# CodyRichter/MLMicroserviceTemplate

Hardware: AMD Instinct MI355X
Metric: requests/sec (whole node) + p50 latency, ResNet-50 bs=32 (higher is better)
Workload: dtype bf16; 1 GPU; model=resnet50-v1.5, global_batch=32, per_gpu_batch=32, image_size=224, parallelism=dp1, backend=fused, concurrent_slots=True, cu_partitions=2, hipgraph=True, inflight=4, numa_bound=True, partition_mode=intra, prestage=False, ranks_consistent=True, dist_backend=none, dist_world=1

## Files before the change

### mlmicroservicetemplate_amd/models/resnet.py

```python
from __future__ import annotations

import math
import os
from dataclasses import dataclass
from typing import Dict, List, Optional, Tuple

import torch
import torch.nn.functional as F

STAGES: Tuple[Tuple[int, int, int, int], ...] = (
    (3, 64, 256, 1),
    (4, 128, 512, 2),
    (6, 256, 1024, 2),
    (3, 512, 2048, 2),
)
IMAGENET_MEAN = (0.485 * 255, 0.456 * 255, 0.406 * 255)
IMAGENET_STD = (0.229 * 255, 0.224 * 255, 0.225 * 255)
NUM_CLASSES = 1000


@dataclass
class ConvSpec:
    name: str
    cin: int
    cout: int
    k: int
    stride: int
    pad: int


def conv_specs() -> List[ConvSpec]:
    specs = [ConvSpec("stem", 3, 64, 7, 2, 3)]
    cin = 64
    for si, (nblocks, mid, cout, stride) in enumerate(STAGES):
        for bi in range(nblocks):
            s = stride if bi == 0 else 1
            p = f"layer{si + 1}.{bi}"
            specs.append(ConvSpec(p + ".conv1", cin, mid, 1, 1, 0))
            specs.append(ConvSpec(p + ".conv2", mid, mid, 3, s, 1))
            specs.append(ConvSpec(p + ".conv3", mid, cout, 1, 1, 0))
            if bi == 0:
                specs.append(ConvSpec(p + ".down", cin, cout, 1, s, 0))
            cin = cout
    return specs


def init_resnet50(seed: int = 0, num_classes: int = NUM_CLASSES) -> Dict[str, torch.Tensor]:
    g = torch.Generator().manual_seed(seed)
    params: Dict[str, torch.Tensor] = {}
    for spec in conv_specs():
        fan_in = spec.cin * spec.k * spec.k
# ... 190 lines not shown
    for s, _hin, ho in conv_shapes(image_size):
        total += 2.0 * ho * ho * s.cout * s.cin * s.k * s.k
    return total + 2.0 * 2048 * NUM_CLASSES


class ResNet50Fused:

    def __init__(self, params: Dict[str, torch.Tensor], device, max_batch: int = 256,
                 tuning: Optional[Dict[str, Tuple[int, int]]] = None, image_size: int = 224):
        from .. import ops

        self.ops = ops
        self.device = torch.device(device)
        self.image_size = image_size
        self.tuning = dict(tuning or {})
        self.specs = {s.name: s for s in conv_specs()}
        self.w: Dict[str, torch.Tensor] = {}
        self.b: Dict[str, torch.Tensor] = {}
        for s in conv_specs():
            scale, bias = fold_bn(params, s.name)
            w = params[s.name + ".w"] * scale.view(-1, 1, 1, 1)
            self.w[s.name] = ops.pack_conv_weight(w).to(self.device)
            self.b[s.name] = bias.to(device=self.device, dtype=torch.float32).contiguous()
        self.dual_w: Dict[str, torch.Tensor] = {}
        self.dual_b: Dict[str, torch.Tensor] = {}
        for si, (_nb, _m, _c, _s) in enumerate(STAGES):
            p0 = f"layer{si + 1}.0"
            w3, wd = self.w[p0 + ".conv3"], self.w[p0 + ".down"]
            self.dual_w[p0] = torch.cat([w3.reshape(w3.shape[0], -1), wd.reshape(wd.shape[0], -1)], 1).contiguous()
            self.dual_b[p0] = (self.b[p0 + ".conv3"] + self.b[p0 + ".down"]).contiguous()
        self.fuse_down = True
        self.chain = os.environ.get("MLS_CHAIN", "1") != "0"
        self.chain_skip: set = {b for b in os.environ.get("MLS_CHAIN_SKIP", "").split(",") if b}
        self.chain_l3 = os.environ.get("MLS_CHAIN_L3", "0") == "1"
        if os.environ.get("MLS_CHAIN_L2_CW"):
            ops.set_chain_l2_cw(int(os.environ["MLS_CHAIN_L2_CW"]))
        if os.environ.get("MLS_CHAIN_L2_BM"):
            ops.lib().mls_chain_set_l2_bm(int(os.environ["MLS_CHAIN_L2_BM"]))
        if os.environ.get("MLS_CHAIN_VARIANT"):
            ops.lib().mls_chain_set_variant(int(os.environ["MLS_CHAIN_VARIANT"]))
        self.fuse_stem = image_size == 224 and os.environ.get("MLS_FUSED_STEM", "1") != "0"
        self.fuse_stem_conv1 = os.environ.get("MLS_STEM_CONV1", "0") == "1"
        self.fc_w = params["fc.w"].to(device=self.device, dtype=torch.bfloat16).contiguous()
        self.fc_b = params["fc.b"].to(device=self.device, dtype=torch.float32).contiguous()
        self.num_classes = self.fc_w.shape[0]
        self.mean = IMAGENET_MEAN
        self.std = IMAGENET_STD
        self.max_batch = max_batch
        self._ws = ops.StreamWorkspace(self._workspace_bytes(max_batch) // 4 + 1, self.device)
        self.fuse_head = os.environ.get("MLS_FUSED_HEAD", "1") != "0"
        self._pool = ops.StreamWorkspace(max_batch * self.fc_w.shape[1], self.device, zero=True)

    @property
    def workspace(self) -> torch.Tensor:
        return self._ws.get()

    @torch.no_grad()
    def update_params(self, params: Dict[str, torch.Tensor]) -> None:
        from .. import ops

        for s in conv_specs():
            scale, bias = fold_bn(params, s.name)
            w = ops.pack_conv_weight(params[s.name + ".w"] * scale.view(-1, 1, 1, 1))
            self.w[s.name].copy_(w)
            self.b[s.name].copy_(bias)
        for si in range(len(STAGES)):
# ... 21 lines not shown
        return self.ops.gemm_heuristic(M, N, K)

    def _workspace_bytes(self, batch: int) -> int:
        need = 0
        for b in sorted({1, 2, 4, 8, 16, 32, 64, 128, 256, batch}):
            if b > batch:
                continue
            for name, M, N, K in self.layer_gemm_shapes(b):
                cfg, sk = self._plan(name, M, N, K)
                if cfg in self.ops.PIPE_CFGS:
                    sk = sk % 16 or 1
                if sk > 1:
                    need = max(need, sk * M * N * 4)
        return max(need, batch * NUM_CLASSES * 4, 1 << 20)

    def _conv(self, x, name, act, residual=None, pad=None):
        s = self.specs[name]
        cfg, sk = self.tuning.get(name, (0, 0))
        return self.ops.conv2d_nhwc(x, self.w[name], self.b[name], kernel=s.k, stride=s.stride,
                                    pad=s.pad if pad is None else pad,
                                    residual=residual, act=act, workspace=self.workspace, cfg=cfg, splitk=sk)


    def _chained(self, p: str, nxt: str, dual: bool) -> bool:
        if not self.chain or p in self.chain_skip:
            return False
        c3 = self.specs[p + ".conv3"]
        k = c3.cin + (self.specs[p + ".down"].cin if dual else 0)
        c1 = self.specs[nxt + ".conv1"]
        shape = (k, c3.cout, c1.cout)
        if shape == (256, 1024, 256) and not self.chain_l3:
            return False
        return c1.k == 1 and c1.stride == 1 and shape in self.ops.CHAIN_SHAPES

    def forward(self, images_u8_nhwc: torch.Tensor) -> torch.Tensor:
        ops = self.ops
        B = images_u8_nhwc.shape[0]
        if self.fuse_head:
            pooled = self._trunk(images_u8_nhwc, pool=True)
            _v, _i, logits = ops.fc_head(pooled, self.fc_w, self.fc_b, 0, logits=self._logits_buf(B))
            return logits.to(torch.bfloat16)
        x = self._trunk(images_u8_nhwc, pool=False)
        pooled = ops.avgpool_global_nhwc(x)
        cfg, sk = self.tuning.get("fc", (0, 0))
        return ops.gemm(pooled, self.fc_w, self.fc_b, workspace=self.workspace, cfg=cfg, splitk=sk)

    __call__ = forward

    def _logits_buf(self, B: int) -> torch.Tensor:
        return self.workspace[: B * self.num_classes].view(B, self.num_classes)

    def classify(self, images_u8_nhwc: torch.Tensor, k: int = 5, err: Optional[torch.Tensor] = None):
        if self.fuse_head:
            pooled = self._trunk(images_u8_nhwc, pool=True)
            B = images_u8_nhwc.shape[0]
            vals, idx, _ = self.ops.fc_head(pooled, self.fc_w, self.fc_b, k, logits=self._logits_buf(B), err=err)
            return vals, idx
        vals, idx = self.ops.softmax_topk(self.forward(images_u8_nhwc), k)
        if err is not None:
            bad = (err[: idx.shape[0]] != 0).view(-1, 1)
            idx = torch.where(bad, torch.full_like(idx, -1), idx)
            vals = torch.where(bad, torch.full_like(vals, float("nan")), vals)
        return vals, idx

    def _trunk(self, images_u8_nhwc: torch.Tensor, pool: bool) -> torch.Tensor:
        ops = self.ops
        B = images_u8_nhwc.shape[0]
        if B > self.max_batch:
            raise ValueError(f"batch {B} > max_batch {self.max_batch}")
        if self.fuse_stem and self.fuse_stem_conv1:
            x, t1 = ops.stem_pool_u8(images_u8_nhwc, self.w["stem"], self.b["stem"], self.mean, self.std,
                                     conv1_w=self.w["layer1.0.conv1"], conv1_b=self.b["layer1.0.conv1"])
        else:
            if self.fuse_stem:
                x = ops.stem_pool_u8(images_u8_nhwc, self.w["stem"], self.b["stem"], self.mean, self.std)
            else:
                x = ops.normalize_u8(images_u8_nhwc, self.mean, self.std, pad=3)
                x = self._conv(x, "stem", ops.ACT_RELU, pad=0)
                x = ops.maxpool2d_nhwc(x, 3, 2, 1)
            t1 = self._conv(x, "layer1.0.conv1", ops.ACT_RELU)
        blocks = [(si, bi) for si, (nblocks, _m, _c, _s) in enumerate(STAGES) for bi in range(nblocks)]
        for idx, (si, bi) in enumerate(blocks):
            p = f"layer{si + 1}.{bi}"
            nxt = f"layer{blocks[idx + 1][0] + 1}.{blocks[idx + 1][1]}" if idx + 1 < len(blocks) else None
            t2 = self._conv(t1, p + ".conv2", ops.ACT_RELU)
            dual = bi == 0 and self.fuse_down
            if nxt is not None and self._chained(p, nxt, dual):
                w1n, b1n = self.w[nxt + ".conv1"], self.b[nxt + ".conv1"]
                w1n = w1n.reshape(w1n.shape[0], -1)
                if dual:
                    x, t1 = ops.conv1x1_chain(t2, self.dual_w[p], self.dual_b[p], w1n, b1n, a2=x,
                                              stride2=self.specs[p + ".down"].stride)
                else:
                    w3 = self.w[p + ".conv3"]
                    x, t1 = ops.conv1x1_chain(t2, w3.reshape(w3.shape[0], -1), self.b[p + ".conv3"], w1n, b1n,
                                              residual=x)
                continue
            if dual:
                cfg, sk = self.tuning.get(p + ".dual", (0, 0))
                x = ops.conv1x1_dual(t2, x, self.dual_w[p], self.dual_b[p], stride2=self.specs[p + ".down"].stride,
                                     act=ops.ACT_RELU, workspace=self.workspace, cfg=cfg, splitk=sk)
            else:
                identity = self._conv(x, p + ".down", ops.ACT_NONE) if bi == 0 else x
                if nxt is None and pool:
                    pooled = self._pool.get()[: B * self.fc_w.shape[1]].view(B, -1)
                    cfg, _sk = self.tuning.get(p + ".conv3", (0, 0))
                    s3 = self.specs[p + ".conv3"]
                    ops.conv2d_pool(t2, self.w[p + ".conv3"], self.b[p + ".conv3"], pooled, kernel=s3.k,
                                    stride=s3.stride, pad=s3.pad, residual=identity, act=ops.ACT_RELU, cfg=cfg)
                    return pooled
                x = self._conv(t2, p + ".conv3", ops.ACT_RELU, residual=identity)
            if nxt is not None:
                t1 = self._conv(x, nxt + ".conv1", ops.ACT_RELU)
        if pool:
            pooled = self._pool.get()[: B * self.fc_w.shape[1]].view(B, -1)
            pooled.copy_(ops.avgpool_global_nhwc(x).float())
            return pooled
        return x
```

### mlmicroservicetemplate_amd/ops/__init__.py

```python
from __future__ import annotations

from . import _lib
from ._lib import NativeError, available, check, lib, stream_ptr
from ._core import (
    ACT_GELU,
    ACT_NONE,
    ACT_RELU,
    ACT_SILU,
    ACT_SILU_MUL,
    ACT_TANH,
    StreamWorkspace,
    conv_out_hw,
)
from .tables import (
    gemm_plan,
    gemm_tile_plan,
    load_blas_tuning,
    small_m_plan_for,
    tile_cfg_for,
    tile_route_for,
)
from .gemm_ops import (
    FP8_MAX,
    GEMM_TILE_CFGS,
# ... 8 lines not shown
    gemm_tile_ln,
    layernorm_from_partials,
    ln_partials,
    interleave_gate_up,
    pack_skinny,
    pack_skinny_fp8,
    pack_skinny_reference,
    silu_mul_interleaved,
    skinny_fp8,
    mgemm,
    skinny_packed,
    skinny_packed_ar,
    split_counters,
)
from .dispatch import (
    BLAS_MIN_M,
    TILE_MIN_M,
    mgemm_route,
    linear_add_rmsnorm,
    linear,
    linear_ln,
    ln_foldable,
)
from .softmax import (
    softmax_rows,
    softmax_topk,
    topk_large,
)
from .vision import (
    CFG_HALO,
    CFG_HALO_N32,
    CFG_HALO_XL,
    CFG_PIPE,
    CHAIN_SHAPES,
    HALO_CFGS,
    PIPE_CFGS,
    PIPE_VARIANTS,
    avgpool_global_nhwc,
    bn_act,
    conv1x1_chain,
    conv1x1_dual,
    conv2d_nhwc,
    conv2d_pool,
    conv3x3_halo,
    conv3x3_halo_geometry,
    conv3x3_pipe,
    conv3x3_pipe_geometry,
    fc_head,
    maxpool2d_nhwc,
    normalize_u8,
    pack_conv_weight,
    set_chain_l2_cw,
    stem_pool_u8,
)
from .transformer import (
    DecodePartials,
    decode_attention,
    decode_attention_fp8,
    decode_pick,
    embed_layernorm,
    embed_layernorm_packed,
    embedding,
    flash_attention,
    flash_attention_rows,
    kv_append,
    last_rows,
    layernorm,
    prefill_slots,
    rmsnorm,
    rope_,
    rope_kv_,
    rope_kv_fp8_,
    skinny_packed_combine,
    skinny_packed_combine_ar,
)
from .image import (
    IMAGE_CONTAINER_BYTES,
    IMAGE_SCRATCH_PER_IMAGE,
# ... 33 lines not shown
```

### mlmicroservicetemplate_amd/ops/_lib.py

```python
from __future__ import annotations

import ctypes
import os
import threading
from typing import Optional

import torch

from . import build as _build

_c = ctypes
_LOCK = threading.Lock()
_LIB: Optional[ctypes.CDLL] = None

P = _c.c_void_p
I = _c.c_int
L = _c.c_long
F = _c.c_float
SZ = _c.c_size_t
FP = _c.POINTER(_c.c_float)

_SIGS = {
    "mls_conv2d": [P, P, P, P, P, P, P, SZ, I, I, I, I, I, I, I, I, I, I, I, I, P],
    "mls_conv2d_dual": [P, P, P, P, P, P, SZ, I, I, I, I, I, I, I, I, I, I, I, I, P],
    "mls_conv_chain": [P, P, P, P, P, P, P, P, P, I, I, I, I, I, I, I, I, I, I, P],
    "mls_gemm": [P, P, P, P, P, P, P, SZ, I, I, I, I, I, I, P],
    "mls_gemm_heuristic": [I, I, I, _c.POINTER(I), _c.POINTER(I)],
    "mls_gemm_tile": [P, P, P, P, P, I, I, I, I, I, I, I, I, I, P, _c.c_longlong, P, I, P],
    "mls_gemm_tile_pick": [I, I],
    "mls_gemm_tile_ln": [P, P, P, P, P, I, I, I, I, I, P, P, P, P, _c.c_longlong, F, P],
    "mls_gemm_num_cfgs": [],
    "mls_normalize_u8": [P, P, I, I, I, I, FP, FP, P],
    "mls_maxpool2d": [P, P, I, I, I, I, I, I, I, P],
    "mls_stem_pool": [P, P, P, P, I, I, I, FP, FP, P],
    "mls_stem_pool_conv1": [P, P, P, P, I, I, I, FP, FP, P, P, P, P],
    "mls_conv3x3_halo": [P, P, P, P, P, P, SZ, I, I, I, I, I, I, I, I, P],
    "mls_conv3x3_halo_geometry": [I, I, I, _c.POINTER(I), _c.POINTER(I)],
    "mls_conv3x3_halo_geometry_v": [I, I, I, I, _c.POINTER(I), _c.POINTER(I)],
    "mls_conv2d_pool": [P, P, P, P, P, P, P, I, I, I, I, I, I, I, I, I, I, I, I, P],
    "mls_fc_head": [P, P, P, P, P, P, P, I, I, I, I, I, P, _c.c_longlong, P],
    "mls_conv3x3_pipe": [P, P, P, P, P, SZ, I, I, I, I, I, I, I, I, I, P],
    "mls_conv3x3_pipe_geometry": [I, I, I, I, _c.POINTER(I), _c.POINTER(I)],
    "mls_conv3x3_pipe_num_variants": [],
    "mls_avgpool_global": [P, P, I, I, I, P],
    "mls_bn_act": [P, P, P, P, L, I, I, P],
    "mls_silu_mul_interleaved": [P, P, L, I, P],
    "mls_softmax_topk": [P, I, P, P, I, I, I, I, F, P],
    "mls_softmax_rows": [P, P, P, I, I, I, F, P],
    "mls_topk_merge": [P, P, P, P, I, I, I, I, I, I, P],
    "mls_topk_chunks": [P, P, P, I, I, I, I, I, P],
    "mls_layernorm": [P, P, P, P, P, P, L, I, F, I, P],
    "mls_embed_ln": [P, P, P, P, P, P, P, P, L, I, I, I, F, P],
    "mls_embed_ln2": [P, P, I, P, P, P, P, P, P, P, P, L, I, I, I, F, P],
    "mls_embedding": [P, P, P, L, I, I, I, P],
    "mls_prefill_slots": [P, P, P, P, I, I, I, I, I, P, P],
    "mls_last_rows": [P, P, P, I, I, I, P, P, P],
    "mls_rope": [P, P, P, P, L, I, I, I, P],
    "mls_ar_create": [I, I, L, P],
# ... 144 lines not shown
```

### mlmicroservicetemplate_amd/ops/csrc/conv_chain.hip

```cpp
#include "common.h"
#include "fastdiv.h"

namespace {

#define LDS3 __attribute__((address_space(3)))

MLS_DEV void glds16(rsrc_t r, char* lds, int voff, int soff) {
  __builtin_amdgcn_raw_ptr_buffer_load_lds(r, (LDS3 void*)lds, 16, voff, soff, 0, 0);
}

typedef unsigned int u32x4v __attribute__((__vector_size__(16)));

#define CONST4 __attribute__((address_space(4)))

MLS_DEV f32x4 bias4(const float* b, int nt0, int fq) {
  if (!b) return f32x4{0.f, 0.f, 0.f, 0.f};
  const CONST4 f32x4* bp = (const CONST4 f32x4*)(b + nt0);
  const f32x4 b0 = bp[0], b1 = bp[1], b2 = bp[2], b3 = bp[3];
  return fq == 0 ? b0 : fq == 1 ? b1 : fq == 2 ? b2 : b3;
}

struct ChainArgs {
  const bf16* a1;
  const bf16* a2;
  const bf16* w3;
  const float* b3;
  const bf16* res;
  bf16* y;
  const bf16* w1;
  const float* b1;
  bf16* t1;
  int M, Ka, Kb, N1, N2;
  int Ho, Wo, H2, W2, stride2;
  FastDiv fd_howo, fd_wo;
  uint32_t a1_bytes, a2_bytes, w3_bytes, res_bytes, y_bytes, w1_bytes, t1_bytes;
};

template <int CPR>
MLS_DEV int row_swz(int r) {
  if constexpr (CPR == 8) return r & 7;
  else return (r & 1) | ((r >> 1) & 2);
}

template <int BM, int KS, int N1, int N2, int CW, int OCC, bool SW>
__global__ __launch_bounds__(512, OCC) void conv_chain_kernel(const ChainArgs a) {
  constexpr int NW = 8, NT = 512, WM = 4, WN = 2;
  constexpr int WTM = BM / WM, TM = WTM / 16;
  constexpr int TN = CW / WN / 16;
  constexpr int TN2 = N2 / WN / 16;
  constexpr int CPR = CW / 8;
  constexpr int RPP = 64 / CPR;
  constexpr int A1_BYTES = BM * KS * 128;
  constexpr int W3_BYTES = CW * KS * 128;
  constexpr int W1_BYTES = N2 * CW * 2;
  constexpr int R_BYTES = BM * CW * 2;
  constexpr int STAGE = W3_BYTES + W1_BYTES + R_BYTES;
  constexpr int EPI_BYTES = BM * N2 * 2;
  constexpr int RING = A1_BYTES + 2 * STAGE;
  constexpr int LDS_BYTES = RING > EPI_BYTES ? RING : EPI_BYTES;
  constexpr int A1_PW = BM / 8 * KS / NW;
  constexpr int W3_PW = CW / 8 * KS / NW;
  constexpr int W1_PW = N2 / RPP / NW;
  constexpr int R_PW = BM / RPP / NW;
  constexpr int Y_ST = BM * CPR / NT;
  constexpr int T_ST = BM * N2 / 8 / NT;
  constexpr int NJ = N1 / CW;
  static_assert(TM >= 1 && TN >= 1 && TN2 >= 1 && (CW == 64 || CW == 32), "tile");
  static_assert(A1_PW * NW * 8 == BM * KS && W3_PW * NW * 8 == CW * KS, "A1 / W3 DMA split");
  static_assert(W1_PW * NW * RPP == N2 && R_PW * NW * RPP == BM, "W1 / residual DMA split");
  static_assert(Y_ST * NT == BM * CPR && T_ST * NT == BM * N2 / 8, "epilogue split");
  static_assert(LDS_BYTES <= 160 * 1024, "LDS");
  __shared__ __attribute__((aligned(16))) char smem[LDS_BYTES];

  const int tid = threadIdx.x, lane = tid & 63;
  const int wid = __builtin_amdgcn_readfirstlane(tid >> 6);
  const int wm = wid / WN, wn = wid % WN;
  const int fr = lane & 15, fq = lane >> 4;
  const int m0 = xcd_remap(blockIdx.x, gridDim.x) * BM;
  const int K1 = a.Ka + a.Kb, KSA = a.Ka / 64;
  const bool has_res = a.res != nullptr;

  float b3v[SW ? 1 : NJ][TN], b1v[TN2];
  if constexpr (!SW) {
#pragma unroll
    for (int j = 0; j < NJ; ++j)
#pragma unroll
      for (int jn = 0; jn < TN; ++jn) b3v[j][jn] = a.b3 ? a.b3[j * CW + wn * (CW / 2) + jn * 16 + fr] : 0.f;
#pragma unroll
    for (int jn = 0; jn < TN2; ++jn) b1v[jn] = a.b1 ? a.b1[wn * (N2 / 2) + jn * 16 + fr] : 0.f;
  }

  const int r8 = lane >> 3, lc = (lane & 7) ^ r8;
  const int rq = lane / CPR, lq = (lane % CPR) ^ row_swz<CPR>(rq);

  const rsrc_t a1r = make_rsrc(a.a1, a.a1_bytes);
  const rsrc_t a2r = make_rsrc(a.a2, a.a2_bytes);
  const rsrc_t w3r = make_rsrc(a.w3, a.w3_bytes);
  const rsrc_t w1r = make_rsrc(a.w1, a.w1_bytes);
  const rsrc_t rr = make_rsrc(a.res, a.res_bytes);
  const rsrc_t yr = make_rsrc(a.y, a.y_bytes);
  const rsrc_t tr = make_rsrc(a.t1, a.t1_bytes);

  char* const sA1 = smem;
  auto stage_base = [&](int buf) { return smem + A1_BYTES + buf * STAGE; };

#pragma unroll
  for (int i = 0; i < A1_PW; ++i) {
    const int q = wid * A1_PW + i;
    const int s = q / (BM / 8), rb = q - s * (BM / 8);
    const int m = m0 + rb * 8 + r8;
    char* dst = sA1 + q * 1024;
    if (s < KSA) {
      glds16(a1r, dst, m < a.M ? (m * a.Ka + s * 64 + lc * 8) * 2 : OOB, 0);
    } else {
      int off = OOB;
      if (m < a.M) {
        const int b = fastdiv(m, a.fd_howo), rem = m - b * (a.Ho * a.Wo);
        const int oh = fastdiv(rem, a.fd_wo), ow = rem - oh * a.Wo;
        off = (((b * a.H2 + oh * a.stride2) * a.W2 + ow * a.stride2) * a.Kb + (s - KSA) * 64 + lc * 8) * 2;
      }
      glds16(a2r, dst, off, 0);
    }
  }

  auto issue = [&](int j, int buf) {
    char* sW3 = stage_base(buf);
    char* sW1 = sW3 + W3_BYTES;
    char* sR = sW1 + W1_BYTES;
#pragma unroll
    for (int i = 0; i < W3_PW; ++i) {
      const int q = wid * W3_PW + i;
      const int s = q / (CW / 8), rb = q - s * (CW / 8);
      glds16(w3r, sW3 + q * 1024, ((j * CW + rb * 8 + r8) * K1 + s * 64 + lc * 8) * 2, 0);
    }
#pragma unroll
    for (int i = 0; i < W1_PW; ++i) {
      const int q = wid * W1_PW + i;
      glds16(w1r, sW1 + q * 1024, ((q * RPP + rq) * N1 + j * CW + lq * 8) * 2, 0);
    }
    if (has_res) {
#pragma unroll
      for (int i = 0; i < R_PW; ++i) {
        const int q = wid * R_PW + i;
        const int m = m0 + q * RPP + rq;
        glds16(rr, sR + q * 1024, m < a.M ? (m * N1 + j * CW + lq * 8) * 2 : OOB, 0);
      }
    }
  };
  issue(0, 0);

  f32x4 acc2[TM][TN2];
#pragma unroll
  for (int i = 0; i < TM; ++i)
#pragma unroll
    for (int jn = 0; jn < TN2; ++jn) acc2[i][jn] = f32x4{0.f, 0.f, 0.f, 0.f};

#pragma unroll
  for (int j = 0; j < NJ; ++j) {
    if (j == 0) {
      asm volatile("s_waitcnt vmcnt(0)" ::: "memory");
      if constexpr (!SW) {
#pragma unroll
        for (int jj = 0; jj < NJ; ++jj)
#pragma unroll
          for (int jn = 0; jn < TN; ++jn) asm volatile("" ::"v"(b3v[jj][jn]));
#pragma unroll
        for (int jn = 0; jn < TN2; ++jn) asm volatile("" ::"v"(b1v[jn]));
      }
    } else {
      asm volatile("s_waitcnt vmcnt(%0)" ::"n"(Y_ST) : "memory");
    }
    asm volatile("s_waitcnt lgkmcnt(0)" ::: "memory");
    __builtin_amdgcn_s_barrier();
    if (j + 1 < NJ) issue(j + 1, (j + 1) & 1);
    char* sW3 = stage_base(j & 1);
    char* sW1 = sW3 + W3_BYTES;
    char* sR = sW1 + W1_BYTES;

    f32x4 acc1[TM][TN];
#pragma unroll
    for (int i = 0; i < TM; ++i)
// ... 148 lines not shown
    const int row = q / TPR, c = q - (q / TPR) * TPR;
    const uint4 v = *reinterpret_cast<const uint4*>(to + row * N2 + ((c ^ (row & 7)) << 3));
    const int m = m0 + row;
    __builtin_amdgcn_raw_buffer_store_b128(__builtin_bit_cast(u32x4v, v), tr, m < a.M ? (m * a.N2 + c * 8) * 2 : OOB,
                                           0, 0);
  }
}

MLS_DEV void vm_wait(int n) {
#define MLS_VMW(k) \
  case k: asm volatile("s_waitcnt vmcnt(" #k ")" ::: "memory"); break;
  switch (n) {
    MLS_VMW(1) MLS_VMW(2) MLS_VMW(3) MLS_VMW(4) MLS_VMW(5) MLS_VMW(6) MLS_VMW(7) MLS_VMW(8) MLS_VMW(9) MLS_VMW(10)
    MLS_VMW(11) MLS_VMW(12) MLS_VMW(13) MLS_VMW(14) MLS_VMW(15) MLS_VMW(16) MLS_VMW(17) MLS_VMW(18) MLS_VMW(19)
    MLS_VMW(20)
    default: asm volatile("s_waitcnt vmcnt(0)" ::: "memory");
  }
#undef MLS_VMW
}

MLS_DEV uint32_t lds_off(const void* p) { return (uint32_t)(uintptr_t)(LDS3 const char*)p; }
MLS_DEV uint2 lds_ld8_issue(uint32_t off) {
  uint2 v;
  asm volatile("ds_read_b64 %0, %1" : "=v"(v) : "v"(off) : "memory");
  return v;
}
MLS_DEV uint32_t lds_ld2_issue(uint32_t off) {
  uint32_t v;
  asm volatile("ds_read_u16 %0, %1" : "=v"(v) : "v"(off) : "memory");
  return v;
}
template <typename T>
MLS_DEV void lds_landed(T& v) { asm volatile("s_waitcnt lgkmcnt(0)" : "+v"(v)::"memory"); }
MLS_DEV uint4 lds_ld16(uint32_t off) {
  uint4 v;
  asm volatile("ds_read_b128 %0, %1\n\ts_waitcnt lgkmcnt(0)" : "=v"(v) : "v"(off) : "memory");
  return v;
}
MLS_DEV void lds_st8(uint32_t off, uint2 v) { asm volatile("ds_write_b64 %0, %1" ::"v"(off), "v"(v) : "memory"); }
MLS_DEV void lds_st2(uint32_t off, bf16 h) {
  const uint32_t v = __builtin_bit_cast(unsigned short, h);
  asm volatile("ds_write_b16 %0, %1" ::"v"(off), "v"(v) : "memory");
}

template <int BM, int KS, int N1, int N2, int CW, int S, int OCC, bool SW, bool PERS>
__global__ __launch_bounds__(512, OCC) void conv_chain_ring_kernel(const ChainArgs a, const int ntiles) {
  constexpr int NW = 8, NT = 512, WM = 4, WN = 2;
  constexpr int WTM = BM / WM, TM = WTM / 16;
  constexpr int TN = CW / WN / 16;
  constexpr int TN2 = N2 / WN / 16;
  constexpr int CPR = CW / 8;
  constexpr int RPP = 64 / CPR;
  constexpr int NJ = N1 / CW;
  constexpr int A1_BYTES = BM * KS * 128;
  constexpr int W3_BYTES = CW * KS * 128;
  constexpr int W1_BYTES = N2 * CW * 2;
  constexpr int R_BYTES = BM * CW * 2;
  constexpr int EPI_BYTES = BM * N2 * 2;
  constexpr int STAGE = PERS ? R_BYTES : W3_BYTES + W1_BYTES + R_BYTES;
  constexpr int OFF_W3 = (PERS ? 2 : 1) * A1_BYTES;
  constexpr int OFF_W1 = OFF_W3 + (PERS ? NJ * W3_BYTES : 0);
  constexpr int OFF_EPI = OFF_W1 + (PERS ? NJ * W1_BYTES : 0);
  constexpr int OFF_RING = OFF_EPI + (PERS ? EPI_BYTES : 0);
  constexpr int RING_END = OFF_RING + S * STAGE;
  constexpr int LDS_BYTES = RING_END > EPI_BYTES ? RING_END : EPI_BYTES;
  constexpr int A1_P = BM / 8 * KS, W3_P = CW / 8 * KS, W1_P = N2 / RPP, R_P = BM / RPP;
// ... 337 lines not shown
#pragma unroll
          for (int r = 0; r < 4; ++r) {
            const int row = wm * WTM + i * 16 + fq * 4 + r;
            const float e = acc2[i][jn][r];
            lds_st2(lds_off(to + row * N2 + ((((col >> 3) ^ (row & 7))) << 3) + (col & 7)), (bf16)fmaxf(e + bb, 0.f));
          }
      }
    }
    asm volatile("s_waitcnt lgkmcnt(0)" ::: "memory");
    __builtin_amdgcn_s_barrier();
#pragma unroll
    for (int it = 0; it < T_ST; ++it) {
      const int q = tid + it * NT;
      const int row = q / TPR, c = q - (q / TPR) * TPR;
      const uint4 v = lds_ld16(lds_off(to + row * N2 + ((c ^ (row & 7)) << 3)));
      const int m = m0 + row;
      __builtin_amdgcn_raw_buffer_store_b128(__builtin_bit_cast(u32x4v, v), tr,
                                             m < a.M ? (m * a.N2 + c * 8) * 2 : OOB, 0, 0);
    }
    if constexpr (!PERS) break;
    tile = chain_next_tile(tile, G);
    if (tile >= ntiles) break;
    m0 = m0n;
    abuf ^= 1;
    first = false;
#pragma unroll
    for (int i = 0; i < TM; ++i)
#pragma unroll
      for (int jn = 0; jn < TN2; ++jn) acc2[i][jn] = f32x4{0.f, 0.f, 0.f, 0.f};
  }
  if constexpr (PERS) asm volatile("s_waitcnt vmcnt(0)" ::: "memory");
}

template <int KS, int N1, int N2, int CW, int BM = 128>
int launch_chain(const ChainArgs& a, hipStream_t st) {
  constexpr int LDS = BM * KS * 128 + 2 * (CW * KS * 128 + N2 * CW * 2 + BM * CW * 2);
  constexpr int OCC = LDS <= 80 * 1024 ? 4 : 2;
#ifdef MLS_CHAIN_SWAP
  constexpr bool SW = MLS_CHAIN_SWAP;
#else
  constexpr bool SW = KS == 1;
#endif
  hipLaunchKernelGGL((conv_chain_kernel<BM, KS, N1, N2, CW, OCC, SW>), dim3((unsigned)((a.M + BM - 1) / BM)),
                     dim3(512), 0, st, a);
  return (int)hipGetLastError();
}

int g_chain_grid = 0;

template <int BM, int KS, int N1, int N2, int CW, int S, bool PERS>
int launch_ring(const ChainArgs& a, hipStream_t st) {
#ifdef MLS_CHAIN_SWAP
  constexpr bool SW = MLS_CHAIN_SWAP;
#else
  constexpr bool SW = KS == 1;
#endif
  constexpr int LDS = PERS ? 2 * BM * KS * 128 + N1 * KS * 128 + N2 * N1 * 2 + BM * N2 * 2 + S * BM * CW * 2
                            : BM * KS * 128 + S * (CW * KS * 128 + N2 * CW * 2 + BM * CW * 2);
  constexpr int OCC = LDS <= 80 * 1024 ? 4 : 2;
  const int ntiles = (a.M + BM - 1) / BM;
  int grid = ntiles;
  if (PERS) {
    const int cus = mls_num_cus();
    grid = g_chain_grid > 0 ? g_chain_grid : (ntiles < cus ? ntiles : cus);
  }
  hipLaunchKernelGGL((conv_chain_ring_kernel<BM, KS, N1, N2, CW, S, OCC, SW, PERS>), dim3((unsigned)grid), dim3(512), 0,
                     st, a, ntiles);
  return (int)hipGetLastError();
}

int g_chain_cw_l2 = 0;
int g_chain_bm_l2 = 128;
int g_chain_variant = 0;

constexpr bool RING_L1_DUAL = false, RING_L2 = true, RING_L2_OUT = false;

// ... 30 lines not shown
  const long M = a.M;
  const long sizes[7] = {M * Ka * 2, (long)B * H2 * W2 * Kb * 2, (long)N1 * (Ka + Kb) * 2, res ? M * N1 * 2 : 0,
                         M * N1 * 2, (long)N2 * N1 * 2, M * N2 * 2};
  for (long s : sizes)
    if (s >= 0x7fffffffL) return MLS_UNSUPPORTED;
  a.a1_bytes = (uint32_t)sizes[0];
  a.a2_bytes = (uint32_t)sizes[1];
  a.w3_bytes = (uint32_t)sizes[2];
  a.res_bytes = (uint32_t)sizes[3];
  a.y_bytes = (uint32_t)sizes[4];
  a.w1_bytes = (uint32_t)sizes[5];
  a.t1_bytes = (uint32_t)sizes[6];
  const hipStream_t st = (hipStream_t)stream;
  const int ks = (Ka + Kb) / 64;
  if (ks == 1 && N1 == 256 && N2 == 64) return launch_chain<1, 256, 64, 64>(a, st);
  if (ks == 2 && N1 == 256 && N2 == 64)
    return use_ring(RING_L1_DUAL) ? launch_ring<64, 2, 256, 64, 64, 2, true>(a, st)
                                  : launch_chain<2, 256, 64, 64>(a, st);
  if (ks == 1 && N1 == 256 && N2 == 128) return launch_chain<1, 256, 128, 64>(a, st);
  const bool l2_override = g_chain_variant == 0 && (g_chain_bm_l2 == 64 || g_chain_cw_l2 != 0);
  if (ks == 2 && N1 == 512 && N2 == 128) {
    if (!l2_override && use_ring(RING_L2)) return launch_ring<128, 2, 512, 128, 64, 2, false>(a, st);
    if (g_chain_bm_l2 == 64) return launch_chain<2, 512, 128, 64, 64>(a, st);
    return g_chain_cw_l2 == 32 ? launch_chain<2, 512, 128, 32>(a, st) : launch_chain<2, 512, 128, 64>(a, st);
  }
  if (ks == 2 && N1 == 512 && N2 == 256) {
    if (!l2_override && use_ring(RING_L2_OUT)) return launch_ring<128, 2, 512, 256, 32, 3, false>(a, st);
    return g_chain_bm_l2 == 64 ? launch_chain<2, 512, 256, 64, 64>(a, st) : launch_chain<2, 512, 256, 32>(a, st);
  }
  if (ks == 4 && N1 == 1024 && N2 == 256) return launch_chain<4, 1024, 256, 32>(a, st);
  return MLS_UNSUPPORTED;
}

void mls_chain_set_l2_cw(int cw) { g_chain_cw_l2 = (cw == 32 || cw == 64) ? cw : 0; }

void mls_chain_set_l2_bm(int bm) { g_chain_bm_l2 = bm == 64 ? 64 : 128; }


void mls_chain_set_variant(int v) { g_chain_variant = (v == 1 || v == 2) ? v : 0; }

void mls_chain_set_grid(int g) { g_chain_grid = g > 0 ? g : 0; }

}

MLS_DEBUG_EXPORT(conv_chain)
```

### mlmicroservicetemplate_amd/ops/vision.py

```python
from __future__ import annotations

import ctypes
from typing import Optional, Tuple

import torch

from ._lib import check, lib, stream_ptr
from ._core import ACT_NONE, ACT_RELU, _act, _need, _ptr, _workspace_args, conv_out_hw


def pack_conv_weight(w_oihw: torch.Tensor, dtype=torch.bfloat16) -> torch.Tensor:
    co, ci, kh, kw = w_oihw.shape
    w = w_oihw.permute(0, 2, 3, 1)
    if ci == 3 and kh > 1:
        w = torch.nn.functional.pad(w, (0, 1, 0, 8 - kw))
    return w.contiguous().to(dtype)


CFG_HALO = 100


CFG_HALO_N32 = 101


# ... 120 lines not shown
    B, Ho, Wo, Ka = a1.shape
    N1, N2 = w3.shape[0], w1.shape[0]
    if a2 is not None:
        _need(a2, "a2", torch.bfloat16, dev)
        if residual is not None:
            raise ValueError("conv1x1_chain: the dual form has no residual")
        B2, H2, W2, Kb = a2.shape
        if B2 != B or conv_out_hw(H2, W2, 1, stride2, 0) != (Ho, Wo):
            raise ValueError("conv1x1_chain: a2 does not match a1's grid at stride2")
    else:
        H2 = W2 = Kb = 0
    if w3.reshape(N1, -1).shape[1] != Ka + Kb or w1.reshape(N2, -1).shape[1] != N1:
        raise ValueError("conv1x1_chain: weight shapes do not chain")
    if (Ka + Kb, N1, N2) not in CHAIN_SHAPES:
        raise ValueError(f"conv1x1_chain: unsupported shape (K {Ka + Kb}, N1 {N1}, N2 {N2})")
    for name, t, n in (("b3", b3, N1), ("b1", b1, N2)):
        if t is not None:
            _need(t, name, torch.float32, dev)
            if t.numel() != n:
                raise ValueError(f"{name} must have {n} elements")
    if residual is not None:
        _need(residual, "residual", torch.bfloat16, dev)
        if tuple(residual.shape) != (B, Ho, Wo, N1):
            raise ValueError("residual shape mismatch")
    y = torch.empty(B, Ho, Wo, N1, device=dev, dtype=torch.bfloat16) if y_out is None else y_out
    t1 = torch.empty(B, Ho, Wo, N2, device=dev, dtype=torch.bfloat16) if t1_out is None else t1_out
    rc = lib().mls_conv_chain(a1.data_ptr(), _ptr(a2), w3.data_ptr(), _ptr(b3), _ptr(residual), y.data_ptr(),
                              w1.data_ptr(), _ptr(b1), t1.data_ptr(), B, Ho, Wo, Ka, H2, W2, Kb, stride2, N1, N2,
                              stream_ptr(dev))
    check(rc, "mls_conv_chain")
    return y, t1


_MEAN_STD_CACHE = {}


def normalize_u8(images: torch.Tensor, mean, std, pad: int = 0, out: Optional[torch.Tensor] = None) -> torch.Tensor:
    dev = images.device
    _need(images, "images", torch.uint8, dev)
    B, H, W, C = images.shape
    if C != 3:
        raise ValueError("expected 3-channel images")
    shape = (B, H + 2 * pad, W + 2 * pad, 4)
    if out is None:
        out = torch.empty(shape, device=dev, dtype=torch.bfloat16)
    else:
        _need(out, "out", torch.bfloat16, dev)
        if tuple(out.shape) != shape:
            raise ValueError(f"out must be {shape}")
    m = (ctypes.c_float * 3)(*[float(v) for v in mean])
    s = (ctypes.c_float * 3)(*[float(v) for v in std])
    rc = lib().mls_normalize_u8(images.data_ptr(), out.data_ptr(), B, H, W, pad, m, s, stream_ptr(dev))
    check(rc, "mls_normalize_u8")
    return out


def stem_pool_u8(images: torch.Tensor, w: torch.Tensor, bias: torch.Tensor, mean, std,
                 out: Optional[torch.Tensor] = None, conv1_w: Optional[torch.Tensor] = None,
                 conv1_b: Optional[torch.Tensor] = None):
    dev = images.device
    _need(images, "images", torch.uint8, dev)
    _need(w, "w", torch.bfloat16, dev)
    _need(bias, "bias", torch.float32, dev)
    B, H, W, C = images.shape
    if C != 3 or H != 224 or W != 224 or tuple(w.shape) != (64, 7, 8, 4) or bias.numel() != 64:
        raise ValueError("stem_pool_u8: 224x224x3 images, [64,7,8,4] weights, 64 biases")
# ... 195 lines not shown
```

Before: 56920 requests/s.

## Fuse layer1 3x3 conv2 into the conv3/conv1 chain kernel

Adds a C2 variant of the chain kernel that computes the 3x3 conv2 (64->64) for a 128-row tile. It stages a halo strip of the input activation in LDS, streams the nine weight taps through a ring, and writes the ReLU result straight into the A1 LDS buffer before the existing conv3+conv1 chain runs. This is enabled by default for layer1 blocks, which removes a separate conv2 launch and the global write and read of its intermediate. In exchange each tile recomputes halo rows and adds LDS pressure and serial work before the chain's GEMMs.

```diff
diff --git a/mlmicroservicetemplate_amd/models/resnet.py b/mlmicroservicetemplate_amd/models/resnet.py
--- a/mlmicroservicetemplate_amd/models/resnet.py
+++ b/mlmicroservicetemplate_amd/models/resnet.py
@@ -17,6 +17,7 @@
 IMAGENET_MEAN = (0.485 * 255, 0.456 * 255, 0.406 * 255)
 IMAGENET_STD = (0.229 * 255, 0.224 * 255, 0.225 * 255)
 NUM_CLASSES = 1000
+CHAIN_CONV2_DEFAULT = ((64, 256, 64), (0, 256, 64))
 
 
 @dataclass
@@ -273,6 +274,10 @@
         self.fuse_down = True
         self.chain = os.environ.get("MLS_CHAIN", "1") != "0"
         self.chain_skip: set = {b for b in os.environ.get("MLS_CHAIN_SKIP", "").split(",") if b}
+        mode = os.environ.get("MLS_CHAIN_CONV2", "1")
+        self.chain_conv2 = mode != "0"
+        self.chain_conv2_shapes = ops.CHAIN_CONV2_SHAPES if mode == "2" else CHAIN_CONV2_DEFAULT
+        self.chain_conv2_skip: set = {b for b in os.environ.get("MLS_CHAIN_CONV2_SKIP", "").split(",") if b}
         self.chain_l3 = os.environ.get("MLS_CHAIN_L3", "0") == "1"
         if os.environ.get("MLS_CHAIN_L2_CW"):
             ops.set_chain_l2_cw(int(os.environ["MLS_CHAIN_L2_CW"]))
@@ -360,6 +365,15 @@
         if shape == (256, 1024, 256) and not self.chain_l3:
             return False
         return c1.k == 1 and c1.stride == 1 and shape in self.ops.CHAIN_SHAPES
+
+    def _conv2_fused(self, p: str, nxt: str, dual: bool, t1: torch.Tensor) -> bool:
+        if not self.chain_conv2 or p in self.chain_conv2_skip:
+            return False
+        c2, c3 = self.specs[p + ".conv2"], self.specs[p + ".conv3"]
+        kb = self.specs[p + ".down"].cin if dual else 0
+        shape = (kb, c3.cout, self.specs[nxt + ".conv1"].cout)
+        return (c2.k == 3 and c2.stride == 1 and c2.pad == 1 and c2.cin == 64 and c2.cout == 64
+                and shape in self.chain_conv2_shapes and t1.shape[2] <= self.ops.CHAIN_CONV2_MAX_W)
 
     def forward(self, images_u8_nhwc: torch.Tensor) -> torch.Tensor:
         ops = self.ops
@@ -411,9 +425,22 @@
         for idx, (si, bi) in enumerate(blocks):
             p = f"layer{si + 1}.{bi}"
             nxt = f"layer{blocks[idx + 1][0] + 1}.{blocks[idx + 1][1]}" if idx + 1 < len(blocks) else None
+            dual = bi == 0 and self.fuse_down
+            chained = nxt is not None and self._chained(p, nxt, dual)
+            if chained and self._conv2_fused(p, nxt, dual, t1):
+                w1n, b1n = self.w[nxt + ".conv1"], self.b[nxt + ".conv1"]
+                w1n = w1n.reshape(w1n.shape[0], -1)
+                w2, b2 = self.w[p + ".conv2"], self.b[p + ".conv2"]
+                if dual:
+                    x, t1 = ops.conv3x3_chain(t1, w2, b2, self.dual_w[p], self.dual_b[p], w1n, b1n, a2=x,
+                                              stride2=self.specs[p + ".down"].stride)
+                else:
+                    w3 = self.w[p + ".conv3"]
+                    x, t1 = ops.conv3x3_chain(t1, w2, b2, w3.reshape(w3.shape[0], -1), self.b[p + ".conv3"], w1n,
+                                              b1n, residual=x)
+                continue
             t2 = self._conv(t1, p + ".conv2", ops.ACT_RELU)
-            dual = bi == 0 and self.fuse_down
-            if nxt is not None and self._chained(p, nxt, dual):
+            if chained:
                 w1n, b1n = self.w[nxt + ".conv1"], self.b[nxt + ".conv1"]
                 w1n = w1n.reshape(w1n.shape[0], -1)
                 if dual:
diff --git a/mlmicroservicetemplate_amd/ops/__init__.py b/mlmicroservicetemplate_amd/ops/__init__.py
--- a/mlmicroservicetemplate_amd/ops/__init__.py
+++ b/mlmicroservicetemplate_amd/ops/__init__.py
@@ -64,6 +64,8 @@
     CFG_HALO_N32,
     CFG_HALO_XL,
     CFG_PIPE,
+    CHAIN_CONV2_MAX_W,
+    CHAIN_CONV2_SHAPES,
     CHAIN_SHAPES,
     HALO_CFGS,
     PIPE_CFGS,
@@ -76,6 +78,7 @@
     conv2d_pool,
     conv3x3_halo,
     conv3x3_halo_geometry,
+    conv3x3_chain,
     conv3x3_pipe,
     conv3x3_pipe_geometry,
     fc_head,
diff --git a/mlmicroservicetemplate_amd/ops/_lib.py b/mlmicroservicetemplate_amd/ops/_lib.py
--- a/mlmicroservicetemplate_amd/ops/_lib.py
+++ b/mlmicroservicetemplate_amd/ops/_lib.py
@@ -24,6 +24,7 @@
     "mls_conv2d": [P, P, P, P, P, P, P, SZ, I, I, I, I, I, I, I, I, I, I, I, I, P],
     "mls_conv2d_dual": [P, P, P, P, P, P, SZ, I, I, I, I, I, I, I, I, I, I, I, I, P],
     "mls_conv_chain": [P, P, P, P, P, P, P, P, P, I, I, I, I, I, I, I, I, I, I, P],
+    "mls_conv_chain_conv2": [P, P, P, P, P, P, P, P, P, P, P, I, I, I, I, I, I, I, I, I, I, P],
     "mls_gemm": [P, P, P, P, P, P, P, SZ, I, I, I, I, I, I, P],
     "mls_gemm_heuristic": [I, I, I, _c.POINTER(I), _c.POINTER(I)],
     "mls_gemm_tile": [P, P, P, P, P, I, I, I, I, I, I, I, I, I, P, _c.c_longlong, P, I, P],
diff --git a/mlmicroservicetemplate_amd/ops/csrc/conv_chain.hip b/mlmicroservicetemplate_amd/ops/csrc/conv_chain.hip
--- a/mlmicroservicetemplate_amd/ops/csrc/conv_chain.hip
+++ b/mlmicroservicetemplate_amd/ops/csrc/conv_chain.hip
@@ -10,6 +10,11 @@
 }
 
 typedef unsigned int u32x4v __attribute__((__vector_size__(16)));
+
+MLS_DEV uint32_t lds_off(const void* p);
+MLS_DEV u32x4v lds_ld16_issue(uint32_t off);
+template <typename T>
+MLS_DEV void lds_landed(T& v);
 
 #define CONST4 __attribute__((address_space(4)))
 
@@ -34,6 +39,10 @@
   int Ho, Wo, H2, W2, stride2;
   FastDiv fd_howo, fd_wo;
   uint32_t a1_bytes, a2_bytes, w3_bytes, res_bytes, y_bytes, w1_bytes, t1_bytes;
+  const bf16* t1in;
+  const bf16* w2;
+  const float* b2;
+  uint32_t t1in_bytes, w2_bytes;
 };
 
 template <int CPR>
@@ -42,7 +51,7 @@
   else return (r & 1) | ((r >> 1) & 2);
 }
 
-template <int BM, int KS, int N1, int N2, int CW, int OCC, bool SW>
+template <int BM, int KS, int N1, int N2, int CW, int OCC, bool SW, bool C2 = false>
 __global__ __launch_bounds__(512, OCC) void conv_chain_kernel(const ChainArgs a) {
   constexpr int NW = 8, NT = 512, WM = 4, WN = 2;
   constexpr int WTM = BM / WM, TM = WTM / 16;
@@ -59,6 +68,8 @@
   constexpr int RING = A1_BYTES + 2 * STAGE;
   constexpr int LDS_BYTES = RING > EPI_BYTES ? RING : EPI_BYTES;
   constexpr int A1_PW = BM / 8 * KS / NW;
+  constexpr int A1_S0 = C2 ? 1 : 0;
+  constexpr int A1_PWL = BM / 8 * (KS - A1_S0) / NW;
   constexpr int W3_PW = CW / 8 * KS / NW;
   constexpr int W1_PW = N2 / RPP / NW;
   constexpr int R_PW = BM / RPP / NW;
@@ -105,8 +116,8 @@
   auto stage_base = [&](int buf) { return smem + A1_BYTES + buf * STAGE; };
 
 #pragma unroll
-  for (int i = 0; i < A1_PW; ++i) {
-    const int q = wid * A1_PW + i;
+  for (int i = 0; i < A1_PWL; ++i) {
+    const int q = A1_S0 * (BM / 8) + wid * A1_PWL + i;
     const int s = q / (BM / 8), rb = q - s * (BM / 8);
     const int m = m0 + rb * 8 + r8;
     char* dst = sA1 + q * 1024;
@@ -147,6 +158,117 @@
       }
     }
   };
+
+  if constexpr (C2) {
+    constexpr int TAPS = 9, TSLOTS = 4, TAHEAD = 3, SROWS = 256, TNP = 64 / WN / 16;
+    static_assert(BM == 128 && STAGE >= SROWS * 128 && STAGE >= TSLOTS * 8192, "strip / tap ring alias one stage each");
+    char* const sS = stage_base(0);
+    char* const sT = stage_base(1);
+    const rsrc_t t1r = make_rsrc(a.t1in, a.t1in_bytes);
+    const rsrc_t w2r = make_rsrc(a.w2, a.w2_bytes);
+    const int halo = a.Wo + 1;
+#pragma unroll
+    for (int i = 0; i < SROWS / 8 / NW; ++i) {
+      const int q = wid * (SROWS / 8 / NW) + i;
+      const int sr = q * 8 + r8, p = m0 - halo + sr;
+      glds16(t1r, sS + q * 1024, (p >= 0 && p < a.M && sr < BM + 2 * halo) ? (p * 64 + lc * 8) * 2 : OOB, 0);
+    }
+    auto issue_tap = [&](int t) {
+      glds16(w2r, sT + (t % TSLOTS) * 8192 + wid * 1024, (((wid * 8 + r8) * TAPS + t) * 64 + lc * 8) * 2, 0);
+    };
+#pragma unroll
+    for (int t = 0; t < TAHEAD; ++t) issue_tap(t);
+
+    int okm[TM];
+#pragma unroll
+    for (int i = 0; i < TM; ++i) {
+      const int m = m0 + wm * WTM + i * 16 + fr;
+      okm[i] = 0;
+      if (m < a.M) {
+        const int b = fastdiv(m, a.fd_howo), rem = m - b * (a.Ho * a.Wo);
+        const int oh = fastdiv(rem, a.fd_wo), ow = rem - oh * a.Wo;
+#pragma unroll
+        for (int t = 0; t < TAPS; ++t)
+          if ((unsigned)(oh + t / 3 - 1) < (unsigned)a.Ho && (unsigned)(ow + t % 3 - 1) < (unsigned)a.Wo)
+            okm[i] |= 1 << t;
+      }
+    }
+
+    f32x4 accp[TM][TNP];
+#pragma unroll
+    for (int i = 0; i < TM; ++i)
+#pragma unroll
+      for (int jn = 0; jn < TNP; ++jn) accp[i][jn] = f32x4{0.f, 0.f, 0.f, 0.f};
+#pragma unroll
+    for (int t = 0; t < TAPS; ++t) {
+      if (t + 2 < TAPS) asm volatile("s_waitcnt vmcnt(2)" ::: "memory");
+      else if (t + 1 < TAPS) asm volatile("s_waitcnt vmcnt(1)" ::: "memory");
+      else asm volatile("s_waitcnt vmcnt(0)" ::: "memory");
+      asm volatile("s_waitcnt lgkmcnt(0)" ::: "memory");
+      __builtin_amdgcn_s_barrier();
+      if (t + TAHEAD < TAPS) issue_tap(t + TAHEAD);
+      const int shift = halo + (t / 3 - 1) * a.Wo + (t % 3 - 1);
+      const uint32_t oS = lds_off(sS), oT = lds_off(sT + (t % TSLOTS) * 8192);
+      u32x4v av[2][TM], bv[2][TNP];
+#pragma unroll
+      for (int kk = 0; kk < 2; ++kk) {
+        const int ch = fq + 4 * kk;
+#pragma unroll
+        for (int i = 0; i < TM; ++i) {
+          const int r = wm * WTM + i * 16 + fr + shift;
+          av[kk][i] = lds_ld16_issue(oS + (r * 8 + (ch ^ (r & 7))) * 16);
+        }
+#pragma unroll
+        for (int jn = 0; jn < TNP; ++jn) {
+          const int n = wn * 32 + jn * 16 + fr;
+          bv[kk][jn] = lds_ld16_issue(oT + (n * 8 + (ch ^ (n & 7))) * 16);
+        }
+      }
+#pragma unroll
+      for (int kk = 0; kk < 2; ++kk) {
+#pragma unroll
+        for (int i = 0; i < TM; ++i) lds_landed(av[kk][i]);
+#pragma unroll
+        for (int jn = 0; jn < TNP; ++jn) lds_landed(bv[kk][jn]);
+      }
+#pragma unroll
+      for (int kk = 0; kk < 2; ++kk) {
+        bf16x8 af[TM], bfv[TNP];
+#pragma unroll
+        for (int i = 0; i < TM; ++i) {
+          u32x4v v = av[kk][i];
+          if (!((okm[i] >> t) & 1)) v = u32x4v{0u, 0u, 0u, 0u};
+          af[i] = __builtin_bit_cast(bf16x8, v);
+        }
+#pragma unroll
+        for (int jn = 0; jn < TNP; ++jn) bfv[jn] = __builtin_bit_cast(bf16x8, bv[kk][jn]);
+#pragma unroll
+        for (int i = 0; i < TM; ++i)
+#pragma unroll
+          for (int jn = 0; jn < TNP; ++jn)
+            accp[i][jn] = __builtin_amdgcn_mfma_f32_16x16x32_bf16(bfv[jn], af[i], accp[i][jn], 0, 0, 0);
+      }
+    }
+#pragma unroll
+    for (int jn = 0; jn < TNP; ++jn) {
+      const int nt0 = wn * 32 + jn * 16, col = nt0 + fq * 4;
+      const f32x4 bb = bias4(a.b2, nt0, fq);
+#pragma unroll
+      for (int i = 0; i < TM; ++i) {
+        const int row = wm * WTM + i * 16 + fr;
+        bf16x4 q;
+#pragma unroll
+        for (int r = 0; r < 4; ++r) {
+          const float e = accp[i][jn][r];
+          q[r] = (bf16)fmaxf(e + bb[r], 0.f);
+        }
+        *reinterpret_cast<uint2*>(sA1 + row * 128 + (((col >> 3) ^ (row & 7)) << 4) + (col & 7) * 2) =
+            __builtin_bit_cast(uint2, q);
+      }
+    }
+    asm volatile("s_waitcnt lgkmcnt(0)" ::: "memory");
+    __builtin_amdgcn_s_barrier();
+  }
   issue(0, 0);
 
   f32x4 acc2[TM][TN2];
@@ -361,6 +483,11 @@
 }
 template <typename T>
 MLS_DEV void lds_landed(T& v) { asm volatile("s_waitcnt lgkmcnt(0)" : "+v"(v)::"memory"); }
+MLS_DEV u32x4v lds_ld16_issue(uint32_t off) {
+  u32x4v v;
+  asm volatile("ds_read_b128 %0, %1" : "=v"(v) : "v"(off) : "memory");
+  return v;
+}
 MLS_DEV uint4 lds_ld16(uint32_t off) {
   uint4 v;
   asm volatile("ds_read_b128 %0, %1\n\ts_waitcnt lgkmcnt(0)" : "=v"(v) : "v"(off) : "memory");
@@ -764,7 +891,7 @@
   if constexpr (PERS) asm volatile("s_waitcnt vmcnt(0)" ::: "memory");
 }
 
-template <int KS, int N1, int N2, int CW, int BM = 128>
+template <int KS, int N1, int N2, int CW, int BM = 128, bool C2 = false>
 int launch_chain(const ChainArgs& a, hipStream_t st) {
   constexpr int LDS = BM * KS * 128 + 2 * (CW * KS * 128 + N2 * CW * 2 + BM * CW * 2);
   constexpr int OCC = LDS <= 80 * 1024 ? 4 : 2;
@@ -773,7 +900,7 @@
 #else
   constexpr bool SW = KS == 1;
 #endif
-  hipLaunchKernelGGL((conv_chain_kernel<BM, KS, N1, N2, CW, OCC, SW>), dim3((unsigned)((a.M + BM - 1) / BM)),
+  hipLaunchKernelGGL((conv_chain_kernel<BM, KS, N1, N2, CW, OCC, SW, C2>), dim3((unsigned)((a.M + BM - 1) / BM)),
                      dim3(512), 0, st, a);
   return (int)hipGetLastError();
 }
@@ -870,6 +997,53 @@
   return MLS_UNSUPPORTED;
 }
 
+int mls_conv_chain_conv2(const void* t1_in, const void* w2, const float* b2, const void* a2, const void* w3,
+                         const float* b3, const void* res, void* y, const void* w1, const float* b1, void* t1, int B,
+                         int H, int W, int Ka, int H2, int W2, int Kb, int stride2, int N1, int N2, void* stream) {
+  if (B <= 0 || H <= 0 || W <= 0 || Ka <= 0 || Kb < 0 || Kb % 64 || N1 <= 0 || N1 % 64 || N2 <= 0) return MLS_BAD_ARG;
+  if (Kb > 0 && (stride2 < 1 || (H - 1) * stride2 >= H2 || (W - 1) * stride2 >= W2 || res)) return MLS_BAD_ARG;
+  if (Ka != 64 || 2 * (W + 1) + 128 > 256) return MLS_UNSUPPORTED;
+  ChainArgs a{};
+  a.t1in = (const bf16*)t1_in;
+  a.w2 = (const bf16*)w2;
+  a.b2 = b2;
+  a.a2 = (const bf16*)a2;
+  a.w3 = (const bf16*)w3;
+  a.b3 = b3;
+  a.res = (const bf16*)res;
+  a.y = (bf16*)y;
+  a.w1 = (const bf16*)w1;
+  a.b1 = b1;
+  a.t1 = (bf16*)t1;
+  a.Ka = Ka;
+  a.Kb = Kb;
+  a.N1 = N1;
+  a.N2 = N2;
+  a.Ho = H, a.Wo = W, a.H2 = H2, a.W2 = W2, a.stride2 = stride2;
+  a.fd_howo = fastdiv_make((uint32_t)(H * W));
+  a.fd_wo = fastdiv_make((uint32_t)W);
+  const long M = (long)B * H * W;
+  const long sizes[7] = {M * Ka * 2, (long)B * H2 * W2 * Kb * 2, (long)N1 * (Ka + Kb) * 2, res ? M * N1 * 2 : 0,
+                         M * N1 * 2, (long)N2 * N1 * 2, M * N2 * 2};
+  for (long s : sizes)
+    if (s >= 0x7fffffffL) return MLS_UNSUPPORTED;
+  a.M = (int)M;
+  a.t1in_bytes = (uint32_t)sizes[0];
+  a.a2_bytes = (uint32_t)sizes[1];
+  a.w3_bytes = (uint32_t)sizes[2];
+  a.res_bytes = (uint32_t)sizes[3];
+  a.y_bytes = (uint32_t)sizes[4];
+  a.w1_bytes = (uint32_t)sizes[5];
+  a.t1_bytes = (uint32_t)sizes[6];
+  a.w2_bytes = 64 * 9 * 64 * 2;
+  const hipStream_t st = (hipStream_t)stream;
+  const int ks = (Ka + Kb) / 64;
+  if (ks == 1 && N1 == 256 && N2 == 64) return launch_chain<1, 256, 64, 64, 128, true>(a, st);
+  if (ks == 2 && N1 == 256 && N2 == 64) return launch_chain<2, 256, 64, 64, 128, true>(a, st);
+  if (ks == 1 && N1 == 256 && N2 == 128) return launch_chain<1, 256, 128, 64, 128, true>(a, st);
+  return MLS_UNSUPPORTED;
+}
+
 void mls_chain_set_l2_cw(int cw) { g_chain_cw_l2 = (cw == 32 || cw == 64) ? cw : 0; }
 
 void mls_chain_set_l2_bm(int bm) { g_chain_bm_l2 = bm == 64 ? 64 : 128; }
diff --git a/mlmicroservicetemplate_amd/ops/vision.py b/mlmicroservicetemplate_amd/ops/vision.py
--- a/mlmicroservicetemplate_amd/ops/vision.py
+++ b/mlmicroservicetemplate_amd/ops/vision.py
@@ -176,6 +176,53 @@
     return y, t1
 
 
+CHAIN_CONV2_SHAPES = ((0, 256, 64), (64, 256, 64), (0, 256, 128))
+CHAIN_CONV2_MAX_W = 63
+
+
+def conv3x3_chain(t1_in: torch.Tensor, w2: torch.Tensor, b2: Optional[torch.Tensor], w3: torch.Tensor,
+                  b3: Optional[torch.Tensor], w1: torch.Tensor, b1: Optional[torch.Tensor], *,
+                  residual: Optional[torch.Tensor] = None, a2: Optional[torch.Tensor] = None, stride2: int = 1,
+                  y_out: Optional[torch.Tensor] = None, t1_out: Optional[torch.Tensor] = None):
+    dev = t1_in.device
+    for name, t in (("t1_in", t1_in), ("w2", w2), ("w3", w3), ("w1", w1)):
+        _need(t, name, torch.bfloat16, dev)
+    B, H, W, C = t1_in.shape
+    N1, N2 = w3.shape[0], w1.shape[0]
+    if C != 64 or tuple(w2.shape) != (64, 3, 3, 64):
+        raise ValueError("conv3x3_chain: t1_in must be [B,H,W,64] and w2 [64,3,3,64]")
+    Ka = 64
+    if a2 is not None:
+        _need(a2, "a2", torch.bfloat16, dev)
+        if residual is not None:
+            raise ValueError("conv3x3_chain: the dual form has no residual")
+        B2, H2, W2, Kb = a2.shape
+        if B2 != B or conv_out_hw(H2, W2, 1, stride2, 0) != (H, W):
+            raise ValueError("conv3x3_chain: a2 does not match t1_in's grid at stride2")
+    else:
+        H2 = W2 = Kb = 0
+    if w3.reshape(N1, -1).shape[1] != Ka + Kb or w1.reshape(N2, -1).shape[1] != N1:
+        raise ValueError("conv3x3_chain: weight shapes do not chain")
+    if (Kb, N1, N2) not in CHAIN_CONV2_SHAPES or W > CHAIN_CONV2_MAX_W:
+        raise ValueError(f"conv3x3_chain: unsupported shape (Kb {Kb}, N1 {N1}, N2 {N2}, W {W})")
+    for name, t, n in (("b2", b2, 64), ("b3", b3, N1), ("b1", b1, N2)):
+        if t is not None:
+            _need(t, name, torch.float32, dev)
+            if t.numel() != n:
+                raise ValueError(f"{name} must have {n} elements")
+    if residual is not None:
+        _need(residual, "residual", torch.bfloat16, dev)
+        if tuple(residual.shape) != (B, H, W, N1):
+            raise ValueError("residual shape mismatch")
+    y = torch.empty(B, H, W, N1, device=dev, dtype=torch.bfloat16) if y_out is None else y_out
+    t1 = torch.empty(B, H, W, N2, device=dev, dtype=torch.bfloat16) if t1_out is None else t1_out
+    rc = lib().mls_conv_chain_conv2(t1_in.data_ptr(), w2.data_ptr(), _ptr(b2), _ptr(a2), w3.data_ptr(), _ptr(b3),
+                                    _ptr(residual), y.data_ptr(), w1.data_ptr(), _ptr(b1), t1.data_ptr(), B, H, W,
+                                    Ka, H2, W2, Kb, stride2, N1, N2, stream_ptr(dev))
+    check(rc, "mls_conv_chain_conv2")
+    return y, t1
+
+
 _MEAN_STD_CACHE = {}
 
 
```

Result: faster. 59120 requests/s (median of 6 runs) (+3.9%).
